# sajadn/Exemplar-VAE

Measured on AMD Instinct MI355X. Metric: training images/sec, higher is better.
Workload: dtype f32

## Files before the change

### exemplar-vae_amd/csrc/evae_dense.hip

```cpp

#include "evae_gemm_x6.h"
#include "evae_gemm_p6.h"
#include "evae_thin.h"
#include "evae_u8_prepare.h"

namespace evae {

__global__ void gated_bwd_input_kernel(const float* __restrict__ dout, const float* __restrict__ gout,
                                       const float* __restrict__ s, int M, int N, int ldo,
                                       float* __restrict__ dh, float* __restrict__ dg, int ldd) {
  const size_t n = (size_t)M * N;
  size_t i = (size_t)blockIdx.x * blockDim.x + threadIdx.x;
  const size_t stride = (size_t)gridDim.x * blockDim.x;
  for (; i < n; i += stride) {
    const size_t row = i / N, col = i % N;
    const float d = dout[row * (size_t)ldd + col], ov = gout[i], sv = s[i];
    const size_t o = row * (size_t)ldo + col;
    dh[o] = d * sv;
    dg[o] = d * ov * (1.0f - sv);
  }
}

__global__ __launch_bounds__(256) void gated_bwd_input_v4_kernel(const float4* __restrict__ dout, const float4* __restrict__ gout,
                                                                 const float4* __restrict__ s, unsigned nquads, unsigned nq,
// ... 846 lines not shown
__global__ void p6_fill_row_kernel(unsigned char* img, int nks, int row, float value, int k_begin, int k_end) {
  const int k = k_begin + blockIdx.x * blockDim.x + threadIdx.x;
  if (k >= k_end) return;
  unsigned short t0, t1, t2;
  p6_split1(value, t0, t1, t2);
  unsigned short* o = reinterpret_cast<unsigned short*>(img + p6_off(row, k, nks));
  o[0] = t0; o[P6_CHUNK / 2] = t1; o[P6_CHUNK] = t2;
}
extern "C" int evae_p6_fill_row(void* img, int nks, int row, float value, int k_begin, int k_end, evae_stream_t stream_) {
  EVAE_REQUIRE(img && nks > 0 && row >= 0 && k_begin >= 0 && k_end <= nks * P6_KS, "p6_fill_row: bad arguments");
  if (k_end <= k_begin) return EVAE_OK;
  p6_fill_row_kernel<<<cdiv(k_end - k_begin, 256), 256, 0, (hipStream_t)stream_>>>((unsigned char*)img, nks, row, value, k_begin, k_end);
  return check_launch("p6_fill_row_kernel");
}

extern "C" int evae_gemm_p6_applies(int M, int N, int gated) {
  static int on = -1;
  if (on < 0) { const char* e = getenv("EVAE_P6"); on = (e && atoi(e) == 0) ? 0 : 1; }
  return (on && gemm_x6_enabled() && gemm_x6_fills(M, N, gated != 0)) ? 1 : 0;
}

extern "C" int evae_gated_dense_fwd_p6t(const void* xT_img, int x_nks, int M, int K, const void* w_img, const float* bh,
                                        const float* bg, int N, float* out, float* save_s, evae_stream_t stream_) {
  EVAE_REQUIRE(M >= 0 && K > 0 && N > 0, "gated_dense_fwd_p6t: bad sizes M=%d K=%d N=%d", M, K, N);
  if (M == 0) return EVAE_OK;
  EVAE_REQUIRE(xT_img && w_img && out && x_nks >= cdiv(M, 128) * 8, "gated_dense_fwd_p6t: bad arguments (k-steps %d)", x_nks);
  GemmArgs g = {};
  g.ones_col = -1; g.npairs = 1;
  g.A[0] = (const float*)xT_img; g.lda[0] = x_nks; g.B[0] = (const float*)w_img; g.Kc[0] = p6_nks(K) * P6_KS;
  g.M = M; g.N = N; g.bias0 = bh; g.bias1 = bg; g.out0 = out; g.out2 = save_s; g.ldo = N;
  return launch_gemm_p6<EPI_GATED, 128, true>(g, 1, (hipStream_t)stream_, "gated_dense_fwd(p6)");
}

extern "C" int evae_dense_bwd_data_p6t(const void* dyT_img, int dy_nks, int M, int N, const void* wT_img, int K,
                                       const float* out_prev, const float* s_prev, float* dh, float* dg, int ldo, void* u8_img,
                                       int u8_nslab, int u8_mbase, evae_stream_t stream_) {
  EVAE_REQUIRE(M >= 0 && K > 0 && N > 0, "dense_bwd_data_p6t: bad sizes M=%d K=%d N=%d", M, K, N);
  if (M == 0) return EVAE_OK;
  EVAE_REQUIRE(dyT_img && wT_img && dy_nks >= cdiv(M, 128) * 8, "dense_bwd_data_p6t: bad arguments (k-steps %d)", dy_nks);
  const bool gate = out_prev != nullptr;
  EVAE_REQUIRE(u8_img ? (gate && s_prev && (u8_mbase % 8) == 0) : (dh && ldo >= K && (!gate || (s_prev && dg))),
               "dense_bwd_data_p6t: bad outputs");
  hipStream_t stream = (hipStream_t)stream_;
  GemmArgs g = {};
  g.ones_col = -1; g.npairs = 1;
  g.A[0] = (const float*)dyT_img; g.lda[0] = dy_nks; g.B[0] = (const float*)wT_img; g.Kc[0] = p6_nks(N) * P6_KS;
  g.M = M; g.N = K; g.out0 = dh; g.out1 = gate ? dg : nullptr; g.ldo = ldo; g.e0 = out_prev; g.e1 = s_prev;
  g.img = (unsigned short*)u8_img; g.img_nslab = u8_nslab; g.img_mbase = u8_mbase;
  const bool narrow = gemm_x6_pick_bn(M, K) == 64;
  if (u8_img) {
    if (narrow) return launch_gemm_p6<EPI_GATE_BWD_IMG, 64, true>(g, 1, stream, "dense_bwd_data(p6, gate, byte-layer images)");
    return launch_gemm_p6<EPI_GATE_BWD_IMG, 128, true>(g, 1, stream, "dense_bwd_data(p6, gate, byte-layer images)");
  }
  if (gate) {
    if (narrow) return launch_gemm_p6<EPI_GATE_BWD, 64, true>(g, 1, stream, "dense_bwd_data(p6, gate)");
    return launch_gemm_p6<EPI_GATE_BWD, 128, true>(g, 1, stream, "dense_bwd_data(p6, gate)");
  }
  if (narrow) return launch_gemm_p6<EPI_LINEAR, 64, true>(g, 1, stream, "dense_bwd_data(p6)");
  return launch_gemm_p6<EPI_LINEAR, 128, true>(g, 1, stream, "dense_bwd_data(p6)");
}

struct P6WgradPlan { int kc, nz, ksplit, local; };
static P6WgradPlan p6_wgrad_plan(int nks, int N, int K, bool with_db) {
  P6WgradPlan p;
  p.kc = K + (with_db ? 1 : 0);
  const int tiles = cdiv(N, BM) * cdiv(p.kc, 64);
  static int slots = -1, local = -1;
  if (slots < 0) { const char* e = getenv("EVAE_P6_WGRAD_SLOTS"); slots = e ? atoi(e) : 256; }
  if (local < 0) { const char* e = getenv("EVAE_P6_WGRAD_LOCAL"); local = e ? atoi(e) : 16; }
  int nz = std::max(1, std::min(slots / std::max(tiles, 1), nks / 8));
  p.local = 0;
  if (local >= 8 && nz >= 8) {
    const int want = (local >= 16 && tiles * 2 <= 64 && nks / 16 >= 8) ? 16 : 8;
    if (tiles * (want / 8) <= 64) { nz = want; p.local = 1; }
  }
  p.ksplit = cdiv(nks, nz);
  p.nz = cdiv(nks, p.ksplit);
  return p;
}
extern "C" size_t evae_dense_bwd_weight_p6_workspace_bytes(int nks, int N, int K) {
  if (nks <= 0 || N <= 0 || K <= 0) return 256;
  const P6WgradPlan p = p6_wgrad_plan(nks, N, K, true);
// ... 20 lines not shown
```

### exemplar-vae_amd/csrc/evae_gemm_kernel.h

```cpp
#pragma once
#include "evae_gemm_core.h"
#include "evae_p6_image.h"
#include <type_traits>
#include <algorithm>

namespace evae {

struct FastDiv { unsigned mul, sh, one; };
__host__ __device__ __forceinline__ unsigned fdiv(unsigned n, const FastDiv d) {
#ifdef __HIP_DEVICE_COMPILE__
  const unsigned t = __umulhi(d.mul, n);
#else
  const unsigned t = (unsigned)(((unsigned long long)d.mul * n) >> 32);
#endif
  return d.one ? n : (t + ((n - t) >> 1)) >> d.sh;
}
static FastDiv make_fastdiv(unsigned d) {
  FastDiv f = {0u, 0u, 0u};
  if (d <= 1) { f.one = 1; return f; }
  unsigned l = 0;
  while ((1ull << l) < d) ++l;
  f.mul = (unsigned)((((1ull << l) - d) << 32) / d + 1);
  f.sh = l - 1;
  return f;
// ... 359 lines not shown
      float bh = (EPI == EPI_GATED && g.bias0 && nok) ? g.bias0[n] : 0.f;
      float bg = (EPI == EPI_GATED && g.bias1 && nok) ? g.bias1[n] : 0.f;
      EVAE_PIN(bh); EVAE_PIN(bg);
#pragma unroll
      for (int mt = 0; mt < MT; ++mt) {
        float ov[16];
#pragma unroll
        for (int r = 0; r < 16; ++r) {
          const int m = m0 + wr * 32 * MT + mt * 32 + (r & 3) + 8 * (r >> 2) + 4 * lh;
          if (EPI == EPI_GATED) {
            const float h = acc[mt][0][r] + bh;
            const float s = __builtin_amdgcn_rcpf(1.0f + __builtin_amdgcn_exp2f(-1.4426950408889634f * (acc[mt][NT - 1][r] + bg)));
            ov[r] = h * s;
            if (m < g.M && nok) {
              const size_t o = orow(m) * g.ldo + n;
              g.out0[o] = ov[r];
              if (g.out1) g.out1[o] = h;
              if (g.out2) g.out2[o] = s;
            }
          } else if (m < g.M && nok) {
            {
              const size_t plane = (size_t)g.M * g.N;
              const size_t o = (size_t)zslice * 2 * plane + (size_t)m * g.N + n;
              g.out0[o] = acc[mt][0][r];
              g.out0[o + plane] = acc[mt][NT - 1][r];
            }
          }
        }
        if (EPI == EPI_GATED && timg)
          p6_emit_tile(g.tsink, g.tsink.row0 + n, nok, g.tsink.kbase + m0 + wr * 32 * MT + mt * 32, ov, lh);
      }
    }
  } else if constexpr (EPI == EPI_GATE_BWD_IMG) {
#pragma unroll
    for (int nt = 0; nt < NT; ++nt) {
      const int n = n0 + wc * 32 * NT + nt * 32 + l31;
      if (n >= g.N) continue;
      float go[MT][16], sv[MT][16];
#pragma unroll
      for (int mt = 0; mt < MT; ++mt)
#pragma unroll
        for (int r = 0; r < 16; ++r) {
          const int m = m0 + wr * 32 * MT + mt * 32 + (r & 3) + 8 * (r >> 2) + 4 * lh;
          const size_t oe = (size_t)(m < g.M ? m : 0) * g.N + n;
          go[mt][r] = g.e0[oe];
          sv[mt][r] = g.e1[oe];
        }
#pragma unroll
      for (int mt = 0; mt < MT; ++mt)
#pragma unroll
        for (int which = 0; which < 2; ++which) {
          const int cc = which ? g.N + n : n;
          const int c = cc & 127;
          unsigned t[4][3][2];
#pragma unroll
          for (int j = 0; j < 4; ++j) {
#pragma unroll
            for (int q = 0; q < 3; ++q) t[j][q][0] = t[j][q][1] = 0u;
#pragma unroll
            for (int i = 0; i < 4; ++i) {
              const int r = 4 * j + i;
              const int m = m0 + wr * 32 * MT + mt * 32 + 8 * j + 4 * lh + i;
              const float v = acc[mt][nt][r], s_ = sv[mt][r];
              float w = which ? v * go[mt][r] * (1.0f - s_) : v * s_;
              if (m >= g.M) w = 0.f;
              const unsigned u0 = __float_as_uint(w) & 0xFFFF0000u;
              const float r1 = w - __uint_as_float(u0);
              const unsigned u1 = __float_as_uint(r1) & 0xFFFF0000u;
              const float r2 = r1 - __uint_as_float(u1);
              const unsigned u2 = __float_as_uint(r2);
              const int sh = 16 * (i & 1);
              t[j][0][i >> 1] |= (u0 >> 16) << sh; t[j][1][i >> 1] |= (u1 >> 16) << sh; t[j][2][i >> 1] |= (u2 >> 16) << sh;
            }
          }
#pragma unroll
          for (int q2 = 0; q2 < 2; ++q2) {
            const int jk = 2 * q2 + lh;
            const int ml = m0 + wr * 32 * MT + mt * 32 + 8 * jk;
            const int gm = ml + g.img_mbase, slab = gm >> 5, mi = gm & 31;
            char* base = reinterpret_cast<char*>(g.img) + ((size_t)((cc >> 7) * g.img_nslab + slab) * 3 * 128 + c) * 64 +
                         ((((mi >> 3) ^ ((c >> 2) & 3))) << 4);
#pragma unroll
            for (int q = 0; q < 3; ++q) {
              const unsigned s0 = lh ? t[2 * q2][q][0] : t[2 * q2 + 1][q][0];
              const unsigned s1 = lh ? t[2 * q2][q][1] : t[2 * q2 + 1][q][1];
              const unsigned r0 = (unsigned)__shfl_xor((int)s0, 32), r1_ = (unsigned)__shfl_xor((int)s1, 32);
              const unsigned k0 = lh ? t[2 * q2 + 1][q][0] : t[2 * q2][q][0];
              const unsigned k1 = lh ? t[2 * q2 + 1][q][1] : t[2 * q2][q][1];
              const uint4 val = lh ? make_uint4(r0, r1_, k0, k1) : make_uint4(k0, k1, r0, r1_);
              if (ml < g.M) *reinterpret_cast<uint4*>(base + (size_t)q * 128 * 64) = val;
            }
          }
        }
    }
  } else if constexpr (EPI == EPI_GATE_BWD) {
    const bool timg = g.tsink.img != nullptr;
#pragma unroll
    for (int nt = 0; nt < NT; ++nt) {
      const int n = n0 + wc * 32 * NT + nt * 32 + l31;
      const bool nok = n < g.N;
      if (!nok && !timg) continue;
      float go[MT][16], sv[MT][16];
#pragma unroll
      for (int mt = 0; mt < MT; ++mt)
#pragma unroll
        for (int r = 0; r < 16; ++r) {
          const int m = m0 + wr * 32 * MT + mt * 32 + (r & 3) + 8 * (r >> 2) + 4 * lh;
          const size_t oe = (size_t)(m < g.M ? m : 0) * g.N + (nok ? n : 0);
          go[mt][r] = g.e0[oe];
          sv[mt][r] = g.e1[oe];
        }
#pragma unroll
      for (int mt = 0; mt < MT; ++mt) {
        float dhv[16], dgv[16];
#pragma unroll
        for (int r = 0; r < 16; ++r) {
          const int m = m0 + wr * 32 * MT + mt * 32 + (r & 3) + 8 * (r >> 2) + 4 * lh;
          const float v = acc[mt][nt][r], s_ = sv[mt][r];
          dhv[r] = v * s_;
          dgv[r] = v * go[mt][r] * (1.0f - s_);
          if (m < g.M && nok && g.out0) {
            const size_t o = orow(m) * g.ldo + n;
            g.out0[o] = dhv[r];
            g.out1[o] = dgv[r];
          }
        }
// ... 609 lines not shown
```

### exemplar-vae_amd/csrc/evae_gemm_p6.h

```cpp
#pragma once
#include "evae_gemm_kernel.h"

namespace evae {

typedef __bf16 p6_bf16x4 __attribute__((ext_vector_type(4)));
typedef __attribute__((address_space(3))) void* p6_lds_t;
typedef __attribute__((address_space(3))) p6_bf16x4* p6_lds4_t;

constexpr int P6_NS = 3;
constexpr int p6_stage_bytes(int bn) { return P6_TILE + 3 * bn * 32; }
constexpr int p6_lds_bytes(int bn) { return P6_NS * p6_stage_bytes(bn); }

template <int OFF>
__device__ __forceinline__ u32x2 p6_tr_read(unsigned lds_addr) {
  u32x2 r;
  asm volatile("ds_read_b64_tr_b16 %0, %1 offset:%2" : "=v"(r) : "v"(lds_addr), "n"(OFF));
  return r;
}

template <int EPI, int BN_, bool TA = false>
__global__ __launch_bounds__(256) __attribute__((amdgpu_waves_per_eu(2, 2))) void gemm_p6_kernel(const GemmArgs g) {
  constexpr bool GATED = (EPI == EPI_GATED || EPI == EPI_RAW_GATED);
  static_assert(BN_ == 128 || (BN_ == 64 && !GATED), "column tile: 128, or 64 for narrow plain outputs");
  constexpr int NW = 4, MT = 2, NT = BN_ / 64;
  constexpr int SB = p6_stage_bytes(BN_), BOFF = P6_TILE, BPL = BN_ * 32;
  extern __shared__ __attribute__((aligned(16))) float smem[];
  char* const lds = reinterpret_cast<char*>(smem);
  const int ntiles = g.tiles_m * g.tiles_n;
  int tile, zs = blockIdx.z;
  if (g.sk_local > 0) {
    const BlockPlace b = block_place(blockIdx.x);
    const SliceTile st = slice_of_block(b, ntiles);
    tile = st.tile; zs = st.slice;
    if (slice_block_idle(b, ntiles, g.sk_local)) return;
  } else {
    tile = tile_of_block(block_place(blockIdx.x), ntiles);
  }
  const int tm = tile / g.tiles_n, tn = tile - tm * g.tiles_n;
  const int m0 = tm * BM;
  const int n0 = GATED ? tn * 64 : tn * BN_;
  const int tid = threadIdx.x, lane = tid & 63;
  const int wave = __builtin_amdgcn_readfirstlane(tid >> 6);
  const int wr = wave >> 1, wc = wave & 1, l31 = lane & 31, lh = lane >> 5;

  f32x16 acc[MT][NT];
#pragma unroll
  for (int i = 0; i < MT; ++i)
#pragma unroll
    for (int j = 0; j < NT; ++j)
#pragma unroll
      for (int r = 0; r < 16; ++r) acc[i][j][r] = 0.f;

  const int nks = g.Kc[0] / P6_KS;
  int s_begin = 0, s_end = nks;
  if (g.ksplit > 0) {
    s_begin = zs * g.ksplit;
    const int e = s_begin + g.ksplit;
    if (e < s_end) s_end = e;
  }
  const int nst = s_end - s_begin;

  const unsigned a_nms = TA ? (unsigned)g.lda[0] : 0u;
  const unsigned grp = (unsigned)nks * P6_GROUP;
  const char* const abase = reinterpret_cast<const char*>(g.A[0]) + (TA ? (size_t)tm * 8 * P6_GROUP : (size_t)tm * 8 * grp);
  const char* const bbase = reinterpret_cast<const char*>(g.B[0]) + (size_t)(GATED ? tn * 8 : tn * (BN_ / 16)) * grp;
  const rsrc_t rA = make_rsrc(abase, 0x7FFFFFFFu);
  const rsrc_t rB = make_rsrc(bbase, 0x7FFFFFFFu);
  const unsigned voff_a = TA ? 0u : (unsigned)lh * grp + (unsigned)l31 * 16u;
  const unsigned voff_b = (unsigned)lh * grp + (unsigned)l31 * 16u;
  const unsigned voff_ta = (unsigned)lh * P6_GROUP + (unsigned)((((l31 >> 1) ^ (4 * lh)) * 32) + (l31 & 1) * 16);

  constexpr int NPIECE = BN_ == 128 ? 6 : 5;
  auto issue_piece = [&](int ks, int b, int q) {
    const unsigned so = (unsigned)ks * (unsigned)P6_GROUP;
    char* const st = lds + b * SB;
    if (q < 3) {
      if constexpr (TA) {
        __builtin_amdgcn_raw_ptr_buffer_load_lds(rA, (p6_lds_t)(st + q * P6_PLANE + wave * 1024), 16, voff_ta,
                                                 (unsigned)ks * a_nms * (unsigned)P6_GROUP + wave * 2 * P6_GROUP + q * P6_CHUNK, 0, 0);
      } else {
        __builtin_amdgcn_raw_ptr_buffer_load_lds(rA, (p6_lds_t)(st + q * P6_PLANE + wave * 1024), 16, voff_a,
                                                 so + (unsigned)(2 * wave) * grp + q * P6_CHUNK, 0, 0);
      }
    } else if constexpr (BN_ == 128) {
      const int p = q - 3;
      __builtin_amdgcn_raw_ptr_buffer_load_lds(rB, (p6_lds_t)(st + BOFF + p * BPL + wave * 1024), 16, voff_b,
                                               so + (unsigned)(2 * wave) * grp + p * P6_CHUNK, 0, 0);
    } else {
      if (q == 3 || wave < 2) {
        const int idx = q == 3 ? wave : wave + 4, p = idx >> 1, j = idx & 1;
        __builtin_amdgcn_raw_ptr_buffer_load_lds(rB, (p6_lds_t)(st + BOFF + p * BPL + j * 1024), 16, voff_b,
                                                 so + (unsigned)(2 * j) * grp + p * P6_CHUNK, 0, 0);
      }
    }
  };
  auto issue = [&](int ks, int b) {
#pragma unroll
    for (int q = 0; q < NPIECE; ++q) issue_piece(ks, b, q);
// ... 118 lines not shown
    if (nst > 2) issue(s_begin + 2, 2);
    if (nst > 2) wait_steps(I2); else if (nst > 1) wait_steps(I1); else wait_steps(I0);
    __builtin_amdgcn_s_barrier();
    read_all(I0, 0);
    int i = 0, b = 0;
    auto adv = [&]() { ++i; b = b == P6_NS - 1 ? 0 : b + 1; };
    while (i + 4 < nst) {
      iter(I0, T, T, I1, i, b); adv();
      iter(I1, T, T, I1, i, b); adv();
    }
#pragma unroll
    for (int u = 0; u < 2; ++u) {
      if (i < nst) {
        if (i + 3 < nst) iter(I0, T, T, I1, i, b);
        else if (i + 2 < nst) iter(I0, T, F, I1, i, b);
        else if (i + 1 < nst) iter(I0, T, F, I0, i, b);
        else iter(I0, F, F, I0, i, b);
        adv();
      }
      if (i < nst) {
        if (i + 3 < nst) iter(I1, T, T, I1, i, b);
        else if (i + 2 < nst) iter(I1, T, F, I1, i, b);
        else if (i + 1 < nst) iter(I1, T, F, I0, i, b);
        else iter(I1, F, F, I0, i, b);
        adv();
      }
    }
    __syncthreads();
  }
  if (g.dbg == 4) return;
  gemm_epilogue<EPI, BN_, NW, 0>(g, acc, m0, n0, tm, wr, wc, lane, smem, zs);
}

static __global__ __launch_bounds__(256) void p6_pack_rows_kernel(const float* __restrict__ x, const float* __restrict__ x2, int R, int K,
                                                           long long ld, int gated, int rows_img, int nks, unsigned char* __restrict__ img) {
  p6_pack_rows_element((size_t)blockIdx.x * blockDim.x + threadIdx.x, x, x2, R, K, ld, gated, rows_img, nks, img);
}

static __global__ __launch_bounds__(256) void p6_pack_cols_kernel(const float* __restrict__ x, const float* __restrict__ x2, int Kd, int R,
                                                           long long ld, int ones_row, int rows_img, int nks, unsigned char* __restrict__ img) {
  p6_pack_cols_element((size_t)blockIdx.x * blockDim.x + threadIdx.x, x, x2, Kd, R, ld, ones_row, rows_img, nks, img);
}

template <int EPI, int BN_ = 128, bool TA = false>
static int launch_gemm_p6(GemmArgs& g, int nz, hipStream_t stream, const char* what) {
  static bool attr_done = false;
  if (!attr_done) {
    (void)hipFuncSetAttribute((const void*)gemm_p6_kernel<EPI, BN_, TA>, hipFuncAttributeMaxDynamicSharedMemorySize, p6_lds_bytes(BN_));
    attr_done = true;
  }
  constexpr bool GATED = (EPI == EPI_GATED || EPI == EPI_RAW_GATED);
  g.tiles_m = cdiv(g.M, BM);
  g.tiles_n = cdiv(g.N, GATED ? 64 : BN_);
  dim3 grid(tile_grid(g.tiles_m * g.tiles_n), 1, nz);
  if (g.sk_local > 0) {
    if (g.sk_local != nz || g.ksplit <= 0) { set_error("%s: XCD-local split needs sk_local == nz and a split contraction", what); return EVAE_EINVAL; }
    grid = dim3(slice_grid(g.tiles_m * g.tiles_n, nz), 1, 1);
  }
  gemm_p6_kernel<EPI, BN_, TA><<<grid, 256, p6_lds_bytes(BN_), stream>>>(g);
  return check_launch(what);
}

}
```

### exemplar-vae_amd/csrc/evae_tile_map.h

```cpp
#pragma once

#ifdef __HIPCC__
#define EVAE_HD __host__ __device__
#else
#define EVAE_HD
#endif
#define EVAE_HD_INLINE EVAE_HD inline __attribute__((always_inline))

namespace evae {

struct BlockPlace { int xcd, slot; };
EVAE_HD_INLINE BlockPlace block_place(const int id) { return {id & 7, id >> 3}; }

EVAE_HD_INLINE int tile_of_block(const BlockPlace b, const int ntiles) {
  const int qq = ntiles >> 3, rr = ntiles & 7;
  return (b.xcd < rr ? b.xcd * (qq + 1) : rr * (qq + 1) + (b.xcd - rr) * qq) + b.slot;
}
EVAE_HD_INLINE int tile_of_block(const int id, const int ntiles) { return tile_of_block(block_place(id), ntiles); }
inline int tile_grid(const int ntiles) { return ntiles; }

inline int u8_fwd_rounds(const int M, const int tiles_n, const int cus, const int h) {
  const int blocks = ((M + h - 1) / h) * tiles_n;
  return (blocks + cus - 1) / cus;
}
inline int u8_fwd_block_rows(const int M, const int tiles_n, const int cus) {
  if (((M + 255) / 256) * tiles_n < cus) return 128;
  const int r256 = u8_fwd_rounds(M, tiles_n, cus, 256), r448 = u8_fwd_rounds(M, tiles_n, cus, 448);
  return (r448 < r256 && r448 * 448 < r256 * 256) ? 448 : 256;
}

struct UnitSlot { int unit, idx; };
EVAE_HD_INLINE bool unit_block_idle(const BlockPlace b, const int nunits, const int per_unit) {
  const int qq = nunits >> 3, rr = nunits & 7;
  return b.slot / per_unit >= qq + (b.xcd < rr ? 1 : 0);
}
EVAE_HD_INLINE UnitSlot unit_of_block(const BlockPlace b, const int nunits, const int per_unit) {
  const int qq = nunits >> 3, rr = nunits & 7;
  const int ul = b.slot / per_unit;
  return {b.xcd * qq + (b.xcd < rr ? b.xcd : rr) + ul, b.slot - ul * per_unit};
}
inline int unit_grid(const int nunits, const int per_unit) {
  const int longest = (nunits + 7) >> 3, last_xcd = (nunits - 1) & 7;
  return 8 * (per_unit * longest - 1) + last_xcd + 1;
}

struct SliceTile { int tile, slice; };
EVAE_HD_INLINE SliceTile slice_of_block(const BlockPlace b, const int ntiles) {
  const int j = b.slot / ntiles;
  return {b.slot - j * ntiles, b.xcd + 8 * j};
}
EVAE_HD_INLINE bool slice_block_idle(const BlockPlace b, const int ntiles, const int nslices) {
  return slice_of_block(b, ntiles).slice >= nslices;
}
inline int slice_grid(const int ntiles, const int nslices) {
  const int last = nslices - 1;
  return 8 * ((last >> 3) * ntiles + ntiles - 1) + (last & 7) + 1;
}

}
```

### exemplar-vae_amd/evae/_lib.py

```python
import ctypes as C
import os

_HERE = os.path.dirname(os.path.abspath(__file__))
LIB_PATH = os.environ.get("EVAE_LIB_PATH") or os.path.join(os.path.dirname(_HERE), "csrc", "libevae_hip.so")

_p = C.c_void_p
_i = C.c_int
_f = C.c_float
_d = C.c_double
_z = C.c_size_t
_l = C.c_int64
_u = C.c_uint
_q = C.c_uint64


class ConvDesc(C.Structure):
    _fields_ = [(n, C.c_int) for n in ("N", "C", "H", "W", "Co", "KH", "KW", "stride", "pad")]


class WtJob(C.Structure):
    _fields_ = [("w1", C.c_void_p), ("w2", C.c_void_p), ("dst", C.c_void_p), ("N", C.c_int), ("K", C.c_int), ("ldt", C.c_int)]


class CtlJob(C.Structure):
# ... 70 lines not shown
    "evae_log_normal_diag_bwd_hardtanh": (_i, [_p, _p, _p, _p, _f, _f, _p, _i, _i, _p, _p, _p, _p]),
    "evae_dense_bwd_data_wt_bytes": (_z, [_i, _i, _i]),
    "evae_dense_bwd_data_wt_ld": (_i, [_i]),
    "evae_dense_bwd_data_wt": (_i, [_p, _p, _p, _p, _i, _i, _i, _i, _p, _p, _p, _p, _i, _p, _p, _z, _p]),
    "evae_dense_bwd_data_workspace_bytes": (_z, [_i, _i, _i, _i]),
    "evae_dense_bwd_data": (_i, [_p, _p, _p, _p, _i, _i, _i, _i, _p, _p, _p, _p, _i, _p, _z, _p]),
    "evae_dense_bwd_weight_workspace_bytes": (_z, [_i, _i, _i]),
    "evae_dense_bwd_weight": (_i, [_p, _i, _i, _i, _p, _p, _i, _i, _p, _p, _i, _p, _z, _p]),
    "evae_dense_bwd_weight_phased": (_i, [_p, _i, _i, _i, _p, _p, _i, _i, _p, _p, _i, _p, _z, _i, _p]),
    "evae_dense_u8_supported": (_i, [_i, C.c_longlong]),
    "evae_dense_u8_block_rows": (_i, [_i, _i, _i]),
    "evae_dense_u8_prepared_bytes": (_z, [_i, _i]),
    "evae_dense_u8_prepare": (_i, [_p, _p, _i, _i, _p, _z, _p]),
    "evae_gated_dense_fwd_u8": (_i, [_p, _p, _i, _i, C.c_longlong, _f, _p, _p, _p, _i, _p, _p, _p]),
    "evae_dense_bwd_weight_u8_workspace_bytes": (_z, [_i, _i, _i]),
    "evae_dense_bwd_weight_u8": (_i, [_p, _i, _i, C.c_longlong, _p, _p, _i, C.c_longlong, _f, _p, _p, _p, _z, _p]),
    "evae_dense_bwd_weight_u8_phased": (_i, [_p, _i, _i, C.c_longlong, _p, _p, _i, C.c_longlong, _f, _p, _p, _p, _z, _i, _p]),
    "evae_dense_bwd_weight_u8_images": (_i, [_i, _i, _i, C.POINTER(C.c_size_t), C.POINTER(C.c_int)]),
    "evae_broadcast_scalar": (_i, [_p, _p, _i, _p]),
    "evae_sum_small": (_i, [_p, _i, _p, _p]),
    "evae_thin_configure": (_i, [_i]),
    "evae_p6_nks": (_i, [_i]),
    "evae_p6_nks_rows": (_i, [_i]),
    "evae_p6_image_bytes": (_z, [_i, _i]),
    "evae_gemm_p6_applies": (_i, [_i, _i, _i]),
    "evae_p6_pack_rows": (_i, [_p, _p, _i, _i, C.c_longlong, _i, _p, _z, _p]),
    "evae_p6_pack_cols": (_i, [_p, _p, _i, _i, C.c_longlong, _i, _i, _p, _z, _p]),
    "evae_p6_fill_row": (_i, [_p, _i, _i, _f, _i, _i, _p]),
    "evae_gated_dense_fwd_timg": (_i, [_p, _p, _i, _i, _i, _p, _p, _p, _p, _i, _p, _p, _p, _p, _i, _i, _i, _p, _z, _p]),
    "evae_gated_dense_fwd_u8_timg": (_i, [_p, _p, _i, _i, C.c_longlong, _f, _p, _p, _p, _i, _p, _p, _p, _i, _i, _i, _p]),
    "evae_dense_bwd_data_timg": (_i, [_p, _p, _p, _p, _i, _i, _i, _i, _p, _p, _p, _p, _i, _p, _p, _i, _i, _i, _p, _z, _p]),
    "evae_gated_dense_fwd_p6t": (_i, [_p, _i, _i, _i, _p, _p, _p, _i, _p, _p, _p]),
    "evae_dense_bwd_data_p6t": (_i, [_p, _i, _i, _i, _p, _i, _p, _p, _p, _p, _i, _p, _i, _i, _p]),
    "evae_dense_bwd_weight_p6_workspace_bytes": (_z, [_i, _i, _i]),
    "evae_dense_bwd_weight_p6": (_i, [_p, _p, _i, _i, _i, _p, _p, _p, _z, _p]),
    "evae_dense_bwd_data_img": (_i, [_p, _p, _p, _p, _i, _i, _i, _i, _p, _p, _p, _i, _i, _p, _p, _z, _p]),
    "evae_dense_bwd_weight_group": (_i, [_p, _i, _p]),
    "evae_dense_bwd_weight_finish_group": (_i, [_p, _i, _p]),
    "evae_gated_dense_bwd_input": (_i, [_p, _p, _p, _i, _i, _p, _p, _i, _p]),
    "evae_gated_dense_bwd_input_ld": (_i, [_p, _i, _p, _p, _i, _i, _p, _p, _i, _p]),
    "evae_gather_rows": (_i, [_p, _p, _p, _i, _i, _p, _p]),
    "evae_gated_dense_bwd": (_i, [_p, _i, _p, _p, _i, _i, _p, _p, _i, _p, _i, _p, _i, _p, _z, _p]),
    "evae_act_bwd": (_i, [_p, _p, _z, _i, _f, _f, _p, _p]),
    "evae_conv2d_workspace_bytes": (_z, [_p, _i, _i]),
    "evae_conv2d_fwd": (_i, [_p, _p, _p, _p, _p, _p, _i, _f, _f, _p, _p, _p, _p, _z, _p]),
    "evae_conv2d_bwd_data": (_i, [_p, _p, _p, _p, _p, _p, _p, _z, _p]),
    "evae_conv2d_bwd_weight": (_i, [_p, _p, _p, _p, _p, _p, _p, _z, _p]),
    "evae_conv2d_cl_supported": (_i, [_p, _i, _i]),
    "evae_conv2d_cl_dy_stride": (_i, [_i]),
    "evae_conv2d_cl_workspace_bytes": (_z, [_p, _i, _i]),
    "evae_conv2d_cl_fwd": (_i, [_p, _p, _p, _p, _p, _p, _i, _f, _f, _p, _p, _p, _p, _z, _p]),
    "evae_conv2d_cl_bwd_data": (_i, [_p, _p, _p, _p, _p, _p, _z, _p]),
    "evae_conv2d_cl_bwd_weight": (_i, [_p, _p, _p, _i, _p, _p, _p, _z, _p]),
    "evae_gemm_x6_configure": (_i, [_i, _i]),
    "evae_gemm_x6_applies": (_i, [_i, _i, _i]),
    "evae_elu_fwd": (_i, [_p, _z, _p, _p]),
    "evae_causal_attn_max_len": (_i, []),
    "evae_causal_attn_lds_bytes": (_z, [_i, _i]),
    "evae_causal_attn_fwd": (_i, [_p, _p, _p, _i, _i, _i, _i, _f, _q, _q, _p, _p, _p]),
    "evae_causal_attn_bwd": (_i, [_p, _p, _p, _p, _p, _p, _i, _i, _i, _i, _f, _q, _q, _p, _p, _p, _p, _p]),
    "evae_elu_dropout_fwd": (_i, [_p, _z, _f, _q, _q, _p, _p]),
    "evae_elu_dropout_bwd": (_i, [_p, _p, _z, _f, _q, _q, _p, _p]),
    "evae_glu_res_fwd": (_i, [_p, _p, _l, _i, _p, _p]),
    "evae_glu_res_bwd": (_i, [_p, _p, _l, _i, _p, _p]),
    "evae_conv2d_cl_res_supported": (_i, [_p]),
    "evae_conv2d_cl_fwd_res": (_i, [_p, _p, _p, _p, _p, _p, _p, _z, _p]),
# ... 111 lines not shown
```

### include/evae_hip.h

```cpp
#ifndef EVAE_HIP_H
#define EVAE_HIP_H

#include <stddef.h>
#include <stdint.h>

#ifdef __cplusplus
extern "C" {
#endif

#define EVAE_OK 0
#define EVAE_EINVAL (-1)
#define EVAE_EWORKSPACE (-2)
#define EVAE_ELAUNCH (-3)

#define EVAE_ABI_VERSION 1

typedef void* evae_stream_t;

int evae_version(void);
const char* evae_last_error(void);
int evae_ctl_upload(void* d_stage, const void* h_pinned, void* d_ctl, size_t bytes, evae_stream_t up, evae_stream_t step,
                    void* ev_used, void* ev_up);

int evae_host_dedup(const int64_t* draws, int n_draws, int64_t n_rows, int cap, int64_t* rows, int64_t* inv, int64_t* rep, float* mult);
// ... 285 lines not shown
                  float beta_host, int B, float* loss, float* KL, float* means, evae_stream_t stream);
int evae_elbo2_fwd(const float* RE, const float* logq1, const float* logp1, const float* logq2, const float* logp2,
                   const float* beta_dev, float beta_host, int B, float* loss, float* KL, float* means, evae_stream_t stream);
int evae_elbo_bwd(const float* dloss, int n_dloss, const float* dRE, int n_dRE, const float* dKL, int n_dKL,
                  const float* beta_dev, float beta_host, int B, float* cRE, float* cKL, float* neg_cKL,
                  evae_stream_t stream);
int evae_step_stats_add(const float* loss, const float* re, const float* kl, float* step3, float* totals3,
                        evae_stream_t stream);
int evae_thin_configure(int max_rows);
int evae_p6_nks(int K);
int evae_p6_nks_rows(int M);
size_t evae_p6_image_bytes(int rows, int nks);
int evae_gemm_p6_applies(int M, int N, int gated);
int evae_p6_pack_rows(const float* x, const float* x2 , int R, int K, long long ld, int gated, void* img,
                      size_t img_bytes, evae_stream_t stream);
int evae_p6_pack_cols(const float* x, const float* x2 , int Kd, int R, long long ld, int ones_row ,
                      int nks, void* img, size_t img_bytes, evae_stream_t stream);
int evae_p6_fill_row(void* img, int nks, int row, float value, int k_begin, int k_end, evae_stream_t stream);
int evae_gated_dense_fwd_timg(const float* x, const int64_t* rows, int M, int K, int ldx, const float* wh, const float* bh,
                              const float* wg, const float* bg, int N, float* out, float* save_h, float* save_s,
                              void* timg, int t_nks, int t_row0, int t_kbase, void* ws, size_t ws_bytes, evae_stream_t stream);
int evae_gated_dense_fwd_u8_timg(const unsigned char* x, const int64_t* rows, int M, int K, long long ldx, float x_scale,
                                 const void* prepared, const float* bh, const float* bg, int N, float* out, float* save_s,
                                 void* timg, int t_nks, int t_row0, int t_kbase, evae_stream_t stream);
int evae_dense_bwd_data_timg(const float* dy1, const float* w1, const float* dy2, const float* w2, int M, int N, int ldy, int K,
                             const float* out_prev, const float* s_prev, float* dx_or_dh, float* dg, int ldo,
                             const float* wT , void* timg, int t_nks, int t_row0, int t_kbase, void* ws,
                             size_t ws_bytes, evae_stream_t stream);
int evae_gated_dense_fwd_p6t(const void* xT_img, int x_nks, int M, int K, const void* w_img, const float* bh, const float* bg,
                             int N, float* out , float* save_s , evae_stream_t stream);
int evae_dense_bwd_data_p6t(const void* dyT_img, int dy_nks, int M, int N, const void* wT_img, int K, const float* out_prev,
                            const float* s_prev, float* dh, float* dg, int ldo, void* u8_img, int u8_nslab, int u8_mbase,
                            evae_stream_t stream);
size_t evae_dense_bwd_weight_p6_workspace_bytes(int nks, int N, int K);
int evae_dense_bwd_weight_p6(const void* dyT_img, const void* xT_img, int nks, int N, int K, float* dw ,
                             float* db , void* ws, size_t ws_bytes,
                             evae_stream_t stream);
int evae_broadcast_scalar(const float* src, float* dst, int n, evae_stream_t stream);
int evae_sum_small(const float* x, int n, float* out, evae_stream_t stream);
int evae_batch_prologue(const float* data, int64_t ldd, const int64_t* idx, int B, int D, int binarize,
                        const int64_t* seed_ctr , float* x_out, int64_t ldx,
                        float* eps_out , int zdim, evae_stream_t stream);
int evae_batch_prologue_u8(const unsigned char* data, int64_t ldd, const int64_t* idx, int B, int D, int binarize,
                           const int64_t* seed_ctr, float x_div, float* x_out, int64_t ldx, unsigned char* stage, int64_t lds,
                           float* eps_out, int zdim, evae_stream_t stream);
typedef struct { const float* w1; const float* w2; float* dst; int N, K, ldt; } evae_wt_job_t;
int evae_batch_prologue_u8_prepare(const unsigned char* data, int64_t ldd, const int64_t* idx, int B, int D, int binarize,
                                   const int64_t* seed_ctr, float x_div, float* x_out, int64_t ldx, unsigned char* stage,
                                   int64_t lds, float* eps_out, int zdim, const float* wh, const float* wg, int N, int K,
                                   void* prepared, size_t prepared_bytes, const evae_wt_job_t* jobs, int njobs,
                                   evae_stream_t stream);
typedef struct { const void* stage0; const void* stage1; void* ctl; size_t bytes; const int* state; size_t idx_word, seed_word; } evae_ctl_job_t;
typedef struct { const float* x; const float* x2; void* img; size_t img_bytes; long long ld; int cols, R, K, flag, nks; } evae_p6_pack_job_t;
int evae_batch_prologue_u8_step(const unsigned char* data, int64_t ldd, int B, int D, int binarize, float x_div, float* x_out,
                                int64_t ldx, unsigned char* stage, int64_t lds, float* eps_out, int zdim, const float* wh,
                                const float* wg, int N, int K, void* prepared, size_t prepared_bytes, const evae_wt_job_t* jobs,
                                int njobs, const evae_ctl_job_t* ctl, const evae_p6_pack_job_t* packs, int npacks,
                                evae_stream_t stream);
int evae_log_normal_diag_bwd_hardtanh(const float* x, const float* mu, const float* logvar, const float* lv_pre, float lo, float hi,
                                      const float* dout, int B, int zdim, float* dx, float* dmu, float* dlv_pre, evae_stream_t stream);
int evae_bernoulli_ll_fwd(const float* x, const float* mean, int B, int D, float* out,
                          evae_stream_t stream);
int evae_bernoulli_ll_bwd(const float* x, const float* mean, const float* dout, int B, int D,
                          float* dmean, evae_stream_t stream);
int evae_log_logistic256_fwd(const float* x, const float* mean, const float* logvar, int lv_scalar, int B, int D,
                             float* out , evae_stream_t stream);
// ... 30 lines not shown
```

Baseline: 198,400.

## Fit backward-data GEMM column strips with a narrow last tile

Adds a fitted launch for the backward-data GEMM. It tiles columns in 128-wide strips and runs the final strip with a 64-wide tile when only 1-64 columns remain, so that work in a mostly empty full-width tile is not wasted. The kernel body is factored out so both tile widths can run in one grid. The byte-image gate epilogue is reorganised to load gate values per row block across all column tiles. This adds template instances and a new env-controlled mode that is on by default, and it may affect register pressure and instruction cache use.

```diff
diff --git a/exemplar-vae_amd/csrc/evae_dense.hip b/exemplar-vae_amd/csrc/evae_dense.hip
--- a/exemplar-vae_amd/csrc/evae_dense.hip
+++ b/exemplar-vae_amd/csrc/evae_dense.hip
@@ -902,6 +902,17 @@
   return launch_gemm_p6<EPI_GATED, 128, true>(g, 1, (hipStream_t)stream_, "gated_dense_fwd(p6)");
 }
 
+static int p6_fit = -1, p6_fit_last = 0;
+static int p6_fit_mode() {
+  if (p6_fit < 0) { const char* e = getenv("EVAE_P6_FIT"); p6_fit = e ? std::max(0, std::min(2, atoi(e))) : 1; }
+  return p6_fit;
+}
+extern "C" int evae_p6_fit_set(int mode) {
+  if (mode >= 0) p6_fit = std::min(mode, 2);
+  return p6_fit_mode();
+}
+extern "C" int evae_p6_fit_last(void) { return p6_fit_last; }
+
 extern "C" int evae_dense_bwd_data_p6t(const void* dyT_img, int dy_nks, int M, int N, const void* wT_img, int K,
                                        const float* out_prev, const float* s_prev, float* dh, float* dg, int ldo, void* u8_img,
                                        int u8_nslab, int u8_mbase, evae_stream_t stream_) {
@@ -918,6 +929,14 @@
   g.M = M; g.N = K; g.out0 = dh; g.out1 = gate ? dg : nullptr; g.ldo = ldo; g.e0 = out_prev; g.e1 = s_prev;
   g.img = (unsigned short*)u8_img; g.img_nslab = u8_nslab; g.img_mbase = u8_mbase;
   const bool narrow = gemm_x6_pick_bn(M, K) == 64;
+  const int fit = p6_fit_mode();
+  p6_fit_last = 0;
+  if (fit && (fit == 2 || !narrow) && p6_last_strip_cols(K) == 64) {
+    p6_fit_last = 64;
+    if (u8_img) return launch_gemm_p6_fit<EPI_GATE_BWD_IMG, true>(g, stream, "dense_bwd_data(p6, gate, byte-layer images, fitted)");
+    if (gate) return launch_gemm_p6_fit<EPI_GATE_BWD, true>(g, stream, "dense_bwd_data(p6, gate, fitted)");
+    return launch_gemm_p6_fit<EPI_LINEAR, true>(g, stream, "dense_bwd_data(p6, fitted)");
+  }
   if (u8_img) {
     if (narrow) return launch_gemm_p6<EPI_GATE_BWD_IMG, 64, true>(g, 1, stream, "dense_bwd_data(p6, gate, byte-layer images)");
     return launch_gemm_p6<EPI_GATE_BWD_IMG, 128, true>(g, 1, stream, "dense_bwd_data(p6, gate, byte-layer images)");
diff --git a/exemplar-vae_amd/csrc/evae_gemm_kernel.h b/exemplar-vae_amd/csrc/evae_gemm_kernel.h
--- a/exemplar-vae_amd/csrc/evae_gemm_kernel.h
+++ b/exemplar-vae_amd/csrc/evae_gemm_kernel.h
@@ -415,66 +415,77 @@
       }
     }
   } else if constexpr (EPI == EPI_GATE_BWD_IMG) {
-#pragma unroll
-    for (int nt = 0; nt < NT; ++nt) {
-      const int n = n0 + wc * 32 * NT + nt * 32 + l31;
-      if (n >= g.N) continue;
-      float go[MT][16], sv[MT][16];
-#pragma unroll
-      for (int mt = 0; mt < MT; ++mt)
-#pragma unroll
-        for (int r = 0; r < 16; ++r) {
-          const int m = m0 + wr * 32 * MT + mt * 32 + (r & 3) + 8 * (r >> 2) + 4 * lh;
-          const size_t oe = (size_t)(m < g.M ? m : 0) * g.N + n;
-          go[mt][r] = g.e0[oe];
-          sv[mt][r] = g.e1[oe];
-        }
-#pragma unroll
-      for (int mt = 0; mt < MT; ++mt)
-#pragma unroll
-        for (int which = 0; which < 2; ++which) {
-          const int cc = which ? g.N + n : n;
-          const int c = cc & 127;
-          unsigned t[4][3][2];
-#pragma unroll
-          for (int j = 0; j < 4; ++j) {
-#pragma unroll
-            for (int q = 0; q < 3; ++q) t[j][q][0] = t[j][q][1] = 0u;
-#pragma unroll
-            for (int i = 0; i < 4; ++i) {
-              const int r = 4 * j + i;
-              const int m = m0 + wr * 32 * MT + mt * 32 + 8 * j + 4 * lh + i;
-              const float v = acc[mt][nt][r], s_ = sv[mt][r];
-              float w = which ? v * go[mt][r] * (1.0f - s_) : v * s_;
-              if (m >= g.M) w = 0.f;
-              const unsigned u0 = __float_as_uint(w) & 0xFFFF0000u;
-              const float r1 = w - __uint_as_float(u0);
-              const unsigned u1 = __float_as_uint(r1) & 0xFFFF0000u;
-              const float r2 = r1 - __uint_as_float(u1);
-              const unsigned u2 = __float_as_uint(r2);
-              const int sh = 16 * (i & 1);
-              t[j][0][i >> 1] |= (u0 >> 16) << sh; t[j][1][i >> 1] |= (u1 >> 16) << sh; t[j][2][i >> 1] |= (u2 >> 16) << sh;
+    constexpr bool PASSES = MT > 1 && NT > 1;
+    constexpr int NOUT = PASSES ? MT : NT;
+#pragma unroll
+    for (int o = 0; o < NOUT; ++o) {
+      const int mt_lo = PASSES ? o : 0, mt_hi = PASSES ? o + 1 : MT, nt_lo = PASSES ? 0 : o, nt_hi = PASSES ? NT : o + 1;
+      float go[MT][NT][16], sv[MT][NT][16];
+#pragma unroll
+      for (int mt = mt_lo; mt < mt_hi; ++mt)
+#pragma unroll
+        for (int nt = nt_lo; nt < nt_hi; ++nt) {
+          const int n = n0 + wc * 32 * NT + nt * 32 + l31;
+          if (n >= g.N) continue;
+#pragma unroll
+          for (int r = 0; r < 16; ++r) {
+            const int m = m0 + wr * 32 * MT + mt * 32 + (r & 3) + 8 * (r >> 2) + 4 * lh;
+            const size_t oe = (size_t)(m < g.M ? m : 0) * g.N + n;
+            go[mt][nt][r] = g.e0[oe];
+            sv[mt][nt][r] = g.e1[oe];
+          }
+        }
+#pragma unroll
+      for (int nt = nt_lo; nt < nt_hi; ++nt) {
+        const int n = n0 + wc * 32 * NT + nt * 32 + l31;
+        if (n >= g.N) continue;
+#pragma unroll
+        for (int mt = mt_lo; mt < mt_hi; ++mt)
+#pragma unroll
+          for (int which = 0; which < 2; ++which) {
+            const int cc = which ? g.N + n : n;
+            const int c = cc & 127;
+            unsigned t[4][3][2];
+#pragma unroll
+            for (int j = 0; j < 4; ++j) {
+#pragma unroll
+              for (int q = 0; q < 3; ++q) t[j][q][0] = t[j][q][1] = 0u;
+#pragma unroll
+              for (int i = 0; i < 4; ++i) {
+                const int r = 4 * j + i;
+                const int m = m0 + wr * 32 * MT + mt * 32 + 8 * j + 4 * lh + i;
+                const float v = acc[mt][nt][r], s_ = sv[mt][nt][r];
+                float w = which ? v * go[mt][nt][r] * (1.0f - s_) : v * s_;
+                if (m >= g.M) w = 0.f;
+                const unsigned u0 = __float_as_uint(w) & 0xFFFF0000u;
+                const float r1 = w - __uint_as_float(u0);
+                const unsigned u1 = __float_as_uint(r1) & 0xFFFF0000u;
+                const float r2 = r1 - __uint_as_float(u1);
+                const unsigned u2 = __float_as_uint(r2);
+                const int sh = 16 * (i & 1);
+                t[j][0][i >> 1] |= (u0 >> 16) << sh; t[j][1][i >> 1] |= (u1 >> 16) << sh; t[j][2][i >> 1] |= (u2 >> 16) << sh;
+              }
             }
-          }
-#pragma unroll
-          for (int q2 = 0; q2 < 2; ++q2) {
-            const int jk = 2 * q2 + lh;
-            const int ml = m0 + wr * 32 * MT + mt * 32 + 8 * jk;
-            const int gm = ml + g.img_mbase, slab = gm >> 5, mi = gm & 31;
-            char* base = reinterpret_cast<char*>(g.img) + ((size_t)((cc >> 7) * g.img_nslab + slab) * 3 * 128 + c) * 64 +
-                         ((((mi >> 3) ^ ((c >> 2) & 3))) << 4);
-#pragma unroll
-            for (int q = 0; q < 3; ++q) {
-              const unsigned s0 = lh ? t[2 * q2][q][0] : t[2 * q2 + 1][q][0];
-              const unsigned s1 = lh ? t[2 * q2][q][1] : t[2 * q2 + 1][q][1];
-              const unsigned r0 = (unsigned)__shfl_xor((int)s0, 32), r1_ = (unsigned)__shfl_xor((int)s1, 32);
-              const unsigned k0 = lh ? t[2 * q2 + 1][q][0] : t[2 * q2][q][0];
-              const unsigned k1 = lh ? t[2 * q2 + 1][q][1] : t[2 * q2][q][1];
-              const uint4 val = lh ? make_uint4(r0, r1_, k0, k1) : make_uint4(k0, k1, r0, r1_);
-              if (ml < g.M) *reinterpret_cast<uint4*>(base + (size_t)q * 128 * 64) = val;
+#pragma unroll
+            for (int q2 = 0; q2 < 2; ++q2) {
+              const int jk = 2 * q2 + lh;
+              const int ml = m0 + wr * 32 * MT + mt * 32 + 8 * jk;
+              const int gm = ml + g.img_mbase, slab = gm >> 5, mi = gm & 31;
+              char* base = reinterpret_cast<char*>(g.img) + ((size_t)((cc >> 7) * g.img_nslab + slab) * 3 * 128 + c) * 64 +
+                           ((((mi >> 3) ^ ((c >> 2) & 3))) << 4);
+#pragma unroll
+              for (int q = 0; q < 3; ++q) {
+                const unsigned s0 = lh ? t[2 * q2][q][0] : t[2 * q2 + 1][q][0];
+                const unsigned s1 = lh ? t[2 * q2][q][1] : t[2 * q2 + 1][q][1];
+                const unsigned r0 = (unsigned)__shfl_xor((int)s0, 32), r1_ = (unsigned)__shfl_xor((int)s1, 32);
+                const unsigned k0 = lh ? t[2 * q2 + 1][q][0] : t[2 * q2][q][0];
+                const unsigned k1 = lh ? t[2 * q2 + 1][q][1] : t[2 * q2][q][1];
+                const uint4 val = lh ? make_uint4(r0, r1_, k0, k1) : make_uint4(k0, k1, r0, r1_);
+                if (ml < g.M) *reinterpret_cast<uint4*>(base + (size_t)q * 128 * 64) = val;
+              }
             }
           }
-        }
+      }
     }
   } else if constexpr (EPI == EPI_GATE_BWD) {
     const bool timg = g.tsink.img != nullptr;
diff --git a/exemplar-vae_amd/csrc/evae_gemm_p6.h b/exemplar-vae_amd/csrc/evae_gemm_p6.h
--- a/exemplar-vae_amd/csrc/evae_gemm_p6.h
+++ b/exemplar-vae_amd/csrc/evae_gemm_p6.h
@@ -18,27 +18,15 @@
   return r;
 }
 
-template <int EPI, int BN_, bool TA = false>
-__global__ __launch_bounds__(256) __attribute__((amdgpu_waves_per_eu(2, 2))) void gemm_p6_kernel(const GemmArgs g) {
+template <int EPI, int BN_, bool TA>
+__device__ __forceinline__ void gemm_p6_body(const GemmArgs& g, float* const smem, const int tm, const int n0, const int bgrp0,
+                                             const int zs) {
   constexpr bool GATED = (EPI == EPI_GATED || EPI == EPI_RAW_GATED);
   static_assert(BN_ == 128 || (BN_ == 64 && !GATED), "column tile: 128, or 64 for narrow plain outputs");
   constexpr int NW = 4, MT = 2, NT = BN_ / 64;
   constexpr int SB = p6_stage_bytes(BN_), BOFF = P6_TILE, BPL = BN_ * 32;
-  extern __shared__ __attribute__((aligned(16))) float smem[];
   char* const lds = reinterpret_cast<char*>(smem);
-  const int ntiles = g.tiles_m * g.tiles_n;
-  int tile, zs = blockIdx.z;
-  if (g.sk_local > 0) {
-    const BlockPlace b = block_place(blockIdx.x);
-    const SliceTile st = slice_of_block(b, ntiles);
-    tile = st.tile; zs = st.slice;
-    if (slice_block_idle(b, ntiles, g.sk_local)) return;
-  } else {
-    tile = tile_of_block(block_place(blockIdx.x), ntiles);
-  }
-  const int tm = tile / g.tiles_n, tn = tile - tm * g.tiles_n;
   const int m0 = tm * BM;
-  const int n0 = GATED ? tn * 64 : tn * BN_;
   const int tid = threadIdx.x, lane = tid & 63;
   const int wave = __builtin_amdgcn_readfirstlane(tid >> 6);
   const int wr = wave >> 1, wc = wave & 1, l31 = lane & 31, lh = lane >> 5;
@@ -63,7 +51,7 @@
   const unsigned a_nms = TA ? (unsigned)g.lda[0] : 0u;
   const unsigned grp = (unsigned)nks * P6_GROUP;
   const char* const abase = reinterpret_cast<const char*>(g.A[0]) + (TA ? (size_t)tm * 8 * P6_GROUP : (size_t)tm * 8 * grp);
-  const char* const bbase = reinterpret_cast<const char*>(g.B[0]) + (size_t)(GATED ? tn * 8 : tn * (BN_ / 16)) * grp;
+  const char* const bbase = reinterpret_cast<const char*>(g.B[0]) + (size_t)bgrp0 * grp;
   const rsrc_t rA = make_rsrc(abase, 0x7FFFFFFFu);
   const rsrc_t rB = make_rsrc(bbase, 0x7FFFFFFFu);
   const unsigned voff_a = TA ? 0u : (unsigned)lh * grp + (unsigned)l31 * 16u;
@@ -248,6 +236,36 @@
   gemm_epilogue<EPI, BN_, NW, 0>(g, acc, m0, n0, tm, wr, wc, lane, smem, zs);
 }
 
+template <int EPI, int BN_, bool TA = false>
+__global__ __launch_bounds__(256) __attribute__((amdgpu_waves_per_eu(2, 2))) void gemm_p6_kernel(const GemmArgs g) {
+  constexpr bool GATED = (EPI == EPI_GATED || EPI == EPI_RAW_GATED);
+  extern __shared__ __attribute__((aligned(16))) float smem[];
+  const int ntiles = g.tiles_m * g.tiles_n;
+  int tile, zs = blockIdx.z;
+  if (g.sk_local > 0) {
+    const BlockPlace b = block_place(blockIdx.x);
+    const SliceTile st = slice_of_block(b, ntiles);
+    tile = st.tile; zs = st.slice;
+    if (slice_block_idle(b, ntiles, g.sk_local)) return;
+  } else {
+    tile = tile_of_block(block_place(blockIdx.x), ntiles);
+  }
+  const int tm = tile / g.tiles_n, tn = tile - tm * g.tiles_n;
+  gemm_p6_body<EPI, BN_, TA>(g, smem, tm, GATED ? tn * 64 : tn * BN_, GATED ? tn * 8 : tn * (BN_ / 16), zs);
+}
+
+template <int EPI, bool TA>
+__global__ __launch_bounds__(256) __attribute__((amdgpu_waves_per_eu(2, 2))) void gemm_p6_fit_kernel(const GemmArgs g, const int last_cols) {
+  static_assert(EPI != EPI_GATED && EPI != EPI_RAW_GATED, "fitted strips: plain outputs");
+  extern __shared__ __attribute__((aligned(16))) float smem[];
+  const StripTile t = p6_strip_of_tile(tile_of_block(block_place(blockIdx.x), g.tiles_m * g.tiles_n), g.tiles_n);
+  if (last_cols == 64 && t.strip == g.tiles_n - 1) {
+    gemm_p6_body<EPI, 64, TA>(g, smem, t.tm, t.strip * 128, t.strip * 8, 0);
+    return;
+  }
+  gemm_p6_body<EPI, 128, TA>(g, smem, t.tm, t.strip * 128, t.strip * 8, 0);
+}
+
 static __global__ __launch_bounds__(256) void p6_pack_rows_kernel(const float* __restrict__ x, const float* __restrict__ x2, int R, int K,
                                                            long long ld, int gated, int rows_img, int nks, unsigned char* __restrict__ img) {
   p6_pack_rows_element((size_t)blockIdx.x * blockDim.x + threadIdx.x, x, x2, R, K, ld, gated, rows_img, nks, img);
@@ -256,6 +274,12 @@
 static __global__ __launch_bounds__(256) void p6_pack_cols_kernel(const float* __restrict__ x, const float* __restrict__ x2, int Kd, int R,
                                                            long long ld, int ones_row, int rows_img, int nks, unsigned char* __restrict__ img) {
   p6_pack_cols_element((size_t)blockIdx.x * blockDim.x + threadIdx.x, x, x2, Kd, R, ld, ones_row, rows_img, nks, img);
+}
+
+static int p6_dbg() {
+  static int dbg = -1;
+  if (dbg < 0) { const char* e = getenv("EVAE_GEMM_DBG"); dbg = (e && atoi(e) == 4) ? 4 : 0; }
+  return dbg;
 }
 
 template <int EPI, int BN_ = 128, bool TA = false>
@@ -273,8 +297,24 @@
     if (g.sk_local != nz || g.ksplit <= 0) { set_error("%s: XCD-local split needs sk_local == nz and a split contraction", what); return EVAE_EINVAL; }
     grid = dim3(slice_grid(g.tiles_m * g.tiles_n, nz), 1, 1);
   }
+  g.dbg = p6_dbg();
   gemm_p6_kernel<EPI, BN_, TA><<<grid, 256, p6_lds_bytes(BN_), stream>>>(g);
   return check_launch(what);
 }
 
-}
+template <int EPI, bool TA>
+static int launch_gemm_p6_fit(GemmArgs& g, hipStream_t stream, const char* what) {
+  static bool attr_done = false;
+  if (!attr_done) {
+    (void)hipFuncSetAttribute((const void*)gemm_p6_fit_kernel<EPI, TA>, hipFuncAttributeMaxDynamicSharedMemorySize, p6_lds_bytes(128));
+    attr_done = true;
+  }
+  if (g.ksplit != 0 || g.sk_local != 0) { set_error("%s: the fitted launch takes the whole contraction", what); return EVAE_EINVAL; }
+  g.tiles_m = cdiv(g.M, BM);
+  g.tiles_n = p6_strips(g.N);
+  g.dbg = p6_dbg();
+  gemm_p6_fit_kernel<EPI, TA><<<p6_fit_grid(g.tiles_m, g.N), 256, p6_lds_bytes(128), stream>>>(g, p6_last_strip_cols(g.N));
+  return check_launch(what);
+}
+
+}
diff --git a/exemplar-vae_amd/csrc/evae_tile_map.h b/exemplar-vae_amd/csrc/evae_tile_map.h
--- a/exemplar-vae_amd/csrc/evae_tile_map.h
+++ b/exemplar-vae_amd/csrc/evae_tile_map.h
@@ -29,6 +29,18 @@
   return (r448 < r256 && r448 * 448 < r256 * 256) ? 448 : 256;
 }
 
+inline int p6_strips(const int N) { return (N + 127) / 128; }
+inline int p6_last_strip_cols(const int N) {
+  const int rem = N % 128;
+  return (N > 128 && rem >= 1 && rem <= 64) ? 64 : 128;
+}
+struct StripTile { int tm, strip; };
+EVAE_HD_INLINE StripTile p6_strip_of_tile(const int tile, const int strips) {
+  const int tm = tile / strips;
+  return {tm, tile - tm * strips};
+}
+inline int p6_fit_grid(const int tiles_m, const int N) { return tile_grid(tiles_m * p6_strips(N)); }
+
 struct UnitSlot { int unit, idx; };
 EVAE_HD_INLINE bool unit_block_idle(const BlockPlace b, const int nunits, const int per_unit) {
   const int qq = nunits >> 3, rr = nunits & 7;
diff --git a/exemplar-vae_amd/evae/_lib.py b/exemplar-vae_amd/evae/_lib.py
--- a/exemplar-vae_amd/evae/_lib.py
+++ b/exemplar-vae_amd/evae/_lib.py
@@ -126,6 +126,8 @@
     "evae_dense_bwd_data_timg": (_i, [_p, _p, _p, _p, _i, _i, _i, _i, _p, _p, _p, _p, _i, _p, _p, _i, _i, _i, _p, _z, _p]),
     "evae_gated_dense_fwd_p6t": (_i, [_p, _i, _i, _i, _p, _p, _p, _i, _p, _p, _p]),
     "evae_dense_bwd_data_p6t": (_i, [_p, _i, _i, _i, _p, _i, _p, _p, _p, _p, _i, _p, _i, _i, _p]),
+    "evae_p6_fit_set": (_i, [_i]),
+    "evae_p6_fit_last": (_i, []),
     "evae_dense_bwd_weight_p6_workspace_bytes": (_z, [_i, _i, _i]),
     "evae_dense_bwd_weight_p6": (_i, [_p, _p, _i, _i, _i, _p, _p, _p, _z, _p]),
     "evae_dense_bwd_data_img": (_i, [_p, _p, _p, _p, _i, _i, _i, _i, _p, _p, _p, _i, _i, _p, _p, _z, _p]),
diff --git a/include/evae_hip.h b/include/evae_hip.h
--- a/include/evae_hip.h
+++ b/include/evae_hip.h
@@ -341,6 +341,8 @@
 int evae_dense_bwd_data_p6t(const void* dyT_img, int dy_nks, int M, int N, const void* wT_img, int K, const float* out_prev,
                             const float* s_prev, float* dh, float* dg, int ldo, void* u8_img, int u8_nslab, int u8_mbase,
                             evae_stream_t stream);
+int evae_p6_fit_set(int mode);
+int evae_p6_fit_last(void);
 size_t evae_dense_bwd_weight_p6_workspace_bytes(int nks, int N, int K);
 int evae_dense_bwd_weight_p6(const void* dyT_img, const void* xT_img, int nks, int N, int K, float* dw ,
                              float* db , void* ws, size_t ws_bytes,
```

After: 201,100, median of 6. 1.01x the previous value.
